# lambdaclass/lambda_elliptic_curves

Hardware: AMD Instinct MI355X
Metric: NTT elems/sec (Stark252 radix-2, 2^24, forward, bit-exact vs CPU: see 'bit_exact') [+ MSM G1 point-adds/sec under 'msm'] (higher is better)
Workload: dtype u32x8 (256-bit Montgomery, 32-bit limbs)

## Files before the change

### lambda_elliptic_curves_amd/csrc/field.cuh

```cuda
#pragma once
#include <stdint.h>

#if defined(__HIPCC__)
#include <hip/hip_runtime.h>
#define LW_HD __host__ __device__ __forceinline__
#else
#define LW_HD inline
#endif

namespace lw {

struct Stark252 {
    static constexpr int N = 8;
    static constexpr bool LAZY = true;
    static constexpr uint32_t INV = 0xffffffffu;
    static constexpr uint32_t TWO_ADICITY = 192;
    LW_HD static constexpr uint32_t p(int i) {
        constexpr uint32_t t[N] = {0x00000001u, 0x00000000u, 0x00000000u, 0x00000000u, 0x00000000u, 0x00000000u, 0x00000011u, 0x08000000u};
        return t[i];
    }
    LW_HD static constexpr uint32_t one(int i) {
        constexpr uint32_t t[N] = {0xffffffe1u, 0xffffffffu, 0xffffffffu, 0xffffffffu, 0xffffffffu, 0xffffffffu, 0xfffffdf0u, 0x07ffffffu};
        return t[i];
    }
// ... 273 lines not shown
    for (int i = 0; i < M + 2; i++) t[i] = 0;
    uint64_t z = (uint64_t)(0u - F::INV);
    z *= 2 - P[0] * z;
    const uint64_t inv = 0 - z;
    for (int i = 0; i < M; i++) {
        u128 c = 0;
        for (int j = 0; j < M; j++) {
            c += (u128)A[j] * B[i] + t[j];
            t[j] = (uint64_t)c;
            c >>= 64;
        }
        c += t[M];
        t[M] = (uint64_t)c;
        t[M + 1] = (uint64_t)(c >> 64);
        const uint64_t m = t[0] * inv;
        c = ((u128)m * P[0] + t[0]) >> 64;
        for (int j = 1; j < M; j++) {
            c += (u128)m * P[j] + t[j];
            t[j - 1] = (uint64_t)c;
            c >>= 64;
        }
        c += t[M];
        t[M - 1] = (uint64_t)c;
        t[M] = t[M + 1] + (uint64_t)(c >> 64);
    }
    Fe<F> r;
    for (int i = 0; i < M; i++) {
        r.v[2 * i] = (uint32_t)t[i];
        r.v[2 * i + 1] = (uint32_t)(t[i] >> 32);
    }
    return reduce_once<F>(r);
}
#endif

#if defined(__HIP_DEVICE_COMPILE__)
#define LW_MAC_V(A, B) "v_mad_u64_u32 %0, vcc, " A ", " B ", %0\n\tv_addc_co_u32_e32 %1, vcc, 0, %1, vcc\n\t"

__device__ __forceinline__ void mac96_x1(uint64_t &lo, uint32_t &hi, uint32_t a0, uint32_t b0) {
    asm(LW_MAC_V("%2", "%3") : "+v"(lo), "+v"(hi) : "v"(a0), "v"(b0) : "vcc");
}
__device__ __forceinline__ void mac96_x2(uint64_t &lo, uint32_t &hi, uint32_t a0, uint32_t b0, uint32_t a1, uint32_t b1) {
    asm(LW_MAC_V("%2", "%3") LW_MAC_V("%4", "%5") : "+v"(lo), "+v"(hi) : "v"(a0), "v"(b0), "v"(a1), "v"(b1) : "vcc");
}
__device__ __forceinline__ void mac96_x4(uint64_t &lo, uint32_t &hi, uint32_t a0, uint32_t b0, uint32_t a1, uint32_t b1,
                                         uint32_t a2, uint32_t b2, uint32_t a3, uint32_t b3) {
    asm(LW_MAC_V("%2", "%3") LW_MAC_V("%4", "%5") LW_MAC_V("%6", "%7") LW_MAC_V("%8", "%9")
        : "+v"(lo), "+v"(hi)
        : "v"(a0), "v"(b0), "v"(a1), "v"(b1), "v"(a2), "v"(b2), "v"(a3), "v"(b3)
        : "vcc");
}
#define LW_MAC_FIRST(A, B, INIT) "v_mad_u64_u32 %0, vcc, " A ", " B ", " INIT "\n\tv_addc_co_u32_e64 %1, vcc, 0, 0, vcc\n\t"
template <uint32_t C>
__device__ __forceinline__ void mac96_c1(uint64_t &lo, uint32_t &hi, uint32_t m0) {
    if constexpr (C == 0) {
    } else if constexpr (C <= 64) {
        asm(LW_MAC_V("%2", "%3") : "+v"(lo), "+v"(hi) : "v"(m0), "n"(C) : "vcc");
    } else {
        asm(LW_MAC_V("%2", "%3") : "+v"(lo), "+v"(hi) : "v"(m0), "s"(C) : "vcc");
    }
}
template <uint32_t C0, uint32_t C1, uint32_t C2, uint32_t C3>
__device__ __forceinline__ void mac96_s4(uint64_t &lo, uint32_t &hi, uint32_t m0, uint32_t m1, uint32_t m2, uint32_t m3) {
    asm(LW_MAC_V("%2", "%3") LW_MAC_V("%4", "%5") LW_MAC_V("%6", "%7") LW_MAC_V("%8", "%9")
        : "+v"(lo), "+v"(hi)
        : "v"(m0), "s"(C0), "v"(m1), "s"(C1), "v"(m2), "s"(C2), "v"(m3), "s"(C3)
        : "vcc");
}

template <class F, int K, int I, int IEND>
__device__ __forceinline__ void col_ab(uint64_t &lo, uint32_t &hi, const Fe<F> &a, const Fe<F> &b) {
    if constexpr (I + 4 <= IEND) {
        mac96_x4(lo, hi, a.v[I], b.v[K - I], a.v[I + 1], b.v[K - I - 1], a.v[I + 2], b.v[K - I - 2], a.v[I + 3], b.v[K - I - 3]);
        col_ab<F, K, I + 4, IEND>(lo, hi, a, b);
    } else if constexpr (I + 2 <= IEND) {
        mac96_x2(lo, hi, a.v[I], b.v[K - I], a.v[I + 1], b.v[K - I - 1]);
        col_ab<F, K, I + 2, IEND>(lo, hi, a, b);
    } else if constexpr (I + 1 <= IEND) {
        mac96_x1(lo, hi, a.v[I], b.v[K - I]);
    }
}
template <uint32_t C>
constexpr bool lw_is_literal() { return C > 64; }
template <class F, int K, int I, int IEND>
__device__ __forceinline__ void col_mp(uint64_t &lo, uint32_t &hi, const uint32_t (&m)[F::N]) {
    if constexpr (I + 4 <= IEND) {
        if constexpr (lw_is_literal<F::p(K - I)>() && lw_is_literal<F::p(K - I - 1)>() && lw_is_literal<F::p(K - I - 2)>() &&
                      lw_is_literal<F::p(K - I - 3)>()) {
            mac96_s4<F::p(K - I), F::p(K - I - 1), F::p(K - I - 2), F::p(K - I - 3)>(lo, hi, m[I], m[I + 1], m[I + 2], m[I + 3]);
            col_mp<F, K, I + 4, IEND>(lo, hi, m);
        } else {
            mac96_c1<F::p(K - I)>(lo, hi, m[I]);
            col_mp<F, K, I + 1, IEND>(lo, hi, m);
        }
    } else if constexpr (I + 1 <= IEND) {
        mac96_c1<F::p(K - I)>(lo, hi, m[I]);
        col_mp<F, K, I + 1, IEND>(lo, hi, m);
    }
}
template <class F>
struct lw_fused_columns {
    static constexpr bool value = false;
};
template <class F, int K, bool A_LT_P>
struct FusedCol;
template <class F, int K>
struct FusedColS;
#include "mac_chains.inc"

template <class F, int LO, int HI>
constexpr bool lw_all_literal() {
    for (int i = LO; i < HI; i++)
        if (F::p(i) <= 64) return false;
    return true;
}

template <class F, int P, int K>
__device__ __forceinline__ void fips_col(uint64_t init, const Fe<F> *const (&a)[P], const Fe<F> *const (&b)[P], uint32_t (&m)[F::N],
                                         uint32_t (&t)[F::N]) {
    constexpr int N = F::N;
    if constexpr (K == 2 * N - 1) {
        t[N - 1] = (uint32_t)init;
    } else {
        uint64_t lo;
        uint32_t hi;
        if constexpr (K < N) {
            col_ab_first_dispatch<F, K, 0, K + 1>(lo, hi, init, *a[0], *b[0]);
            if constexpr (P > 1) col_ab<F, K, 0, K + 1>(lo, hi, *a[1], *b[1]);
            if constexpr (P > 2) col_ab<F, K, 0, K + 1>(lo, hi, *a[2], *b[2]);
            if constexpr (P > 3) col_ab<F, K, 0, K + 1>(lo, hi, *a[3], *b[3]);
            if constexpr (K >= 1 && lw_all_literal<F, 1, K + 1>()) col_mp_dispatch<F, K, 0, K>(lo, hi, m);
            else col_mp<F, K, 0, K>(lo, hi, m);
            uint32_t mk;
            if constexpr (F::INV == 0xffffffffu) mk = 0u - (uint32_t)lo;
            else mk = (uint32_t)lo * F::INV;
            m[K] = mk;
            mac96_c1<F::p(0)>(lo, hi, mk);
        } else {
            col_ab_first_dispatch<F, K, K - N + 1, 2 * N - 1 - K>(lo, hi, init, *a[0], *b[0]);
            if constexpr (P > 1) col_ab<F, K, K - N + 1, N>(lo, hi, *a[1], *b[1]);
            if constexpr (P > 2) col_ab<F, K, K - N + 1, N>(lo, hi, *a[2], *b[2]);
            if constexpr (P > 3) col_ab<F, K, K - N + 1, N>(lo, hi, *a[3], *b[3]);
            if constexpr (lw_all_literal<F, K - N + 1, N>()) col_mp_dispatch<F, K, K - N + 1, 2 * N - 1 - K>(lo, hi, m);
            else col_mp<F, K, K - N + 1, N>(lo, hi, m);
            t[K - N] = (uint32_t)lo;
        }
        fips_col<F, P, K + 1>((lo >> 32) | ((uint64_t)hi << 32), a, b, m, t);
    }
}
__device__ __forceinline__ void lw_redc_unit(uint32_t &m, uint32_t &mid, uint32_t &top, uint32_t t, uint32_t w1, uint32_t w2) {
    asm("v_sub_co_u32_e32 %0, vcc, 0, %3\n\t"
        "v_addc_co_u32_e32 %1, vcc, 0, %4, vcc\n\t"
        "v_addc_co_u32_e32 %2, vcc, 0, %5, vcc"
        : "=&v"(m), "=&v"(mid), "=v"(top)
        : "v"(t), "v"(w1), "v"(w2)
        : "vcc");
}
__device__ __forceinline__ void lw_redc_unit0(uint32_t &m, uint32_t &mid, uint32_t &top, uint32_t t, uint32_t w1) {
    asm("v_sub_co_u32_e32 %0, vcc, 0, %3\n\t"
        "v_addc_co_u32_e32 %1, vcc, 0, %4, vcc\n\t"
        "v_addc_co_u32_e64 %2, vcc, 0, 0, vcc"
        : "=&v"(m), "=&v"(mid), "=v"(top)
        : "v"(t), "v"(w1)
        : "vcc");
}
template <class F, int K, bool A_LT_P, bool A_SGPR = false>
__device__ __forceinline__ void fips_fused(uint64_t init, const Fe<F> &a, const Fe<F> &b, uint32_t (&m)[F::N], uint32_t (&t)[F::N]) {
    constexpr int N = F::N;
    static_assert(F::p(0) == 1u && F::INV == 0xffffffffu, "fused columns need a unit low limb of the modulus");
    if constexpr (K == 2 * N - 1) {
        t[N - 1] = (uint32_t)init;
    } else {
        uint64_t lo;
        uint32_t hi;
        static_assert(A_LT_P || !A_SGPR, "the scalar-operand columns exist for a < p only");
        if constexpr (A_SGPR) FusedColS<F, K>::run(lo, hi, init, a, b, m);
        else FusedCol<F, K, A_LT_P>::run(lo, hi, init, a, b, m);
        if constexpr (K < N) {
            uint32_t mid, top;
            if constexpr (K == 0) lw_redc_unit0(m[0], mid, top, (uint32_t)lo, (uint32_t)(lo >> 32));
            else lw_redc_unit(m[K], mid, top, (uint32_t)lo, (uint32_t)(lo >> 32), hi);
            fips_fused<F, K + 1, A_LT_P, A_SGPR>(((uint64_t)top << 32) | mid, a, b, m, t);
        } else {
            t[K - N] = (uint32_t)lo;
            fips_fused<F, K + 1, A_LT_P, A_SGPR>((lo >> 32) | ((uint64_t)hi << 32), a, b, m, t);
        }
    }
}
template <class F, bool A_LT_P = false, bool A_SGPR = false>
__device__ __forceinline__ void fips_product(const Fe<F> &a, const Fe<F> &b, uint32_t (&t)[F::N]) {
    uint32_t m[F::N];
    if constexpr (lw_fused_columns<F>::value) {
        fips_fused<F, 0, A_LT_P, A_SGPR>(0ull, a, b, m, t);
    } else {
        const Fe<F> *const pa[1] = {&a}, *const pb[1] = {&b};
        fips_col<F, 1, 0>(0ull, pa, pb, m, t);
    }
}
template <class F>
__device__ __forceinline__ Fe<F> fe_mul_gfx9(const Fe<F> &a, const Fe<F> &b) {
    constexpr int N = F::N;
    uint32_t t[N];
    fips_product<F>(a, b, t);
    Fe<F> r;
#pragma unroll
    for (int i = 0; i < N; i++) r.v[i] = t[i];
    return reduce_once<F>(r);
}
#endif

template <class F>
LW_HD Fe<F> fe_mul(const Fe<F> &a, const Fe<F> &b) {
#if defined(__HIP_DEVICE_COMPILE__)
    return fe_mul_gfx9<F>(a, b);
#elif defined(LW_HOST_MUL64)
    return fe_mul_host64<F>(a, b);
#else
    return fe_mul_portable<F>(a, b);
#endif
}

template <class F>
LW_HD Fe<F> fe_sqr(const Fe<F> &a) { return fe_mul<F>(a, a); }

template <class F>
LW_HD Fe<F> fe_neg_raw(const Fe<F> &a) {
    uint32_t pk[F::N];
    limbs_kp<F, 0>(pk);
    Fe<F> r;
    limbs_sub<F::N>(r.v, pk, a.v);
    return r;
}
template <class F>
LW_HD Fe<F> fe_neg_raw_2p(const Fe<F> &a) {
    uint32_t pk[F::N];
    limbs_kp<F, 1>(pk);
    Fe<F> r;
    limbs_sub<F::N>(r.v, pk, a.v);
    return r;
}
template <class F, int P, int KSUM = P>
LW_HD Fe<F> fe_dot(const Fe<F> *const (&a)[P], const Fe<F> *const (&b)[P]) {
    static_assert(P >= 1 && P <= 4, "fe_dot: 1..4 products");
    static_assert(KSUM >= P, "fe_dot: KSUM counts every product at least once");
    static_assert((uint64_t)KSUM * ((uint64_t)F::p(F::N - 1) + 1) <= (1ull << 32), "fe_dot: sum of products would exceed 2p after reduction");
#if defined(__HIP_DEVICE_COMPILE__)
    constexpr int N = F::N;
    uint32_t m[N], t[N];
    fips_col<F, P, 0>(0ull, a, b, m, t);
    Fe<F> r;
#pragma unroll
    for (int i = 0; i < N; i++) r.v[i] = t[i];
    return reduce_once<F>(r);
#else
    static_assert(KSUM == P, "fe_dot: unreduced operands are a device-code feature");
    Fe<F> acc = fe_mul<F>(reduce_once<F>(*a[0]), *b[0]);
    for (int q = 1; q < P; q++) acc = fe_add<F>(acc, fe_mul<F>(reduce_once<F>(*a[q]), *b[q]));
    return acc;
#endif
}

template <class F, int LOGK>
LW_HD Fe<F> fe_cond_sub_kp(const Fe<F> &a) {
    constexpr int N = F::N;
    uint32_t kp[N];
    limbs_kp<F, LOGK>(kp);
    Fe<F> d;
    const uint32_t borrow = limbs_sub<N>(d.v, a.v, kp);
    Fe<F> r;
#pragma unroll
    for (int i = 0; i < N; i++) r.v[i] = borrow ? a.v[i] : d.v[i];
    return r;
}
LW_HD Fe<Stark252> fe_reduce_full(const Fe<Stark252> &x) {
    const uint32_t q = x.v[7] >> 27;
    const uint32_t z = lw_k(0u);
    const uint32_t sub[8] = {q, z, z, z, z, z, 17u * q, q << 27};
    Fe<Stark252> d;
    const uint32_t borrow = limbs_sub<8>(d.v, x.v, sub);
    uint32_t pm[8];
    limbs_p_masked<Stark252>(pm, 0u - borrow);
    Fe<Stark252> r;
    limbs_add<8>(r.v, d.v, pm);
    return r;
}
template <class F>
LW_HD Fe<F> fe_reduce_full(const Fe<F> &x) { return reduce_once<F>(x); }

template <class F>
LW_HD Fe<F> fe_add_raw(const Fe<F> &a, const Fe<F> &b) {
    Fe<F> s;
    limbs_add<F::N>(s.v, a.v, b.v);
    return s;
}
template <class F>
LW_HD Fe<F> fe_add2p_sub_raw(const Fe<F> &a, const Fe<F> &b) {
    constexpr int N = F::N;
    uint32_t kp[N];
    limbs_kp<F, 1>(kp);
    Fe<F> d, r;
    limbs_sub<N>(d.v, a.v, b.v);
    limbs_add<N>(r.v, d.v, kp);
    return r;
}
template <class F>
LW_HD Fe<F> fe_mul_lazy(const Fe<F> &a, const Fe<F> &b) {
#if defined(__HIP_DEVICE_COMPILE__)
    constexpr int N = F::N;
    uint32_t t[N];
    fips_product<F, true>(a, b, t);
    Fe<F> r;
#pragma unroll
    for (int i = 0; i < N; i++) r.v[i] = t[i];
    return r;
#else
    return fe_mul_portable_raw<F>(a, b);
#endif
}
template <class F>
LW_HD Fe<F> fe_mul_lazy_uniform(const Fe<F> &a, const Fe<F> &b) {
#if defined(__HIP_DEVICE_COMPILE__)
    constexpr int N = F::N;
    uint32_t t[N];
    fips_product<F, true, lw_fused_columns<F>::value>(a, b, t);
    Fe<F> r;
#pragma unroll
    for (int i = 0; i < N; i++) r.v[i] = t[i];
    return r;
#else
    return fe_mul_portable_raw<F>(a, b);
#endif
}

template <class F>
LW_HD Fe<F> fe_pow_u64(Fe<F> base, uint64_t e) {
    Fe<F> r = Fe<F>::one();
    while (e) {
        if (e & 1) r = fe_mul<F>(r, base);
        base = fe_sqr<F>(base);
        e >>= 1;
    }
    return r;
}

template <class F>
LW_HD Fe<F> fe_inv(const Fe<F> &a) {
    constexpr int N = F::N;
    uint32_t e[N];
    uint64_t borrow = 2;
#pragma unroll
    for (int i = 0; i < N; i++) {
        uint64_t t = (uint64_t)F::p(i) - borrow;
        e[i] = (uint32_t)t;
        borrow = (t >> 32) & 1;
    }
    Fe<F> r = Fe<F>::one();
    for (int i = N - 1; i >= 0; i--) {
        for (int bit = 31; bit >= 0; bit--) {
            r = fe_sqr<F>(r);
            if ((e[i] >> bit) & 1) r = fe_mul<F>(r, a);
        }
    }
    return r;
}

template <class F>
LW_HD constexpr int fe_modulus_bits() {
    int top = 0;
    for (int b = 0; b < 32; b++)
        if ((F::p(F::N - 1) >> b) & 1u) top = b + 1;
    return 32 * (F::N - 1) + top;
}
template <int N>
LW_HD uint32_t bingcd_update_ab(uint32_t (&x)[N], uint32_t (&y)[N], int32_t f, int32_t g, int32_t h, int32_t k) {
    int64_t cx = 0, cy = 0;
    uint32_t wx[N + 1], wy[N + 1];
#pragma unroll
    for (int i = 0; i < N; i++) {
        const int64_t zx = (int64_t)x[i] * f + (int64_t)y[i] * g + cx;
        const int64_t zy = (int64_t)x[i] * h + (int64_t)y[i] * k + cy;
        wx[i] = (uint32_t)zx;
        wy[i] = (uint32_t)zy;
        cx = zx >> 32;
        cy = zy >> 32;
    }
    wx[N] = (uint32_t)cx;
    wy[N] = (uint32_t)cy;
    const uint32_t nx = (uint32_t)((uint64_t)cx >> 63), ny = (uint32_t)((uint64_t)cy >> 63);
    uint32_t carx = nx, cary = ny;
#pragma unroll
    for (int i = 0; i < N; i++) {
        uint32_t rx = (wx[i] >> 30) | (wx[i + 1] << 2), ry = (wy[i] >> 30) | (wy[i + 1] << 2);
        rx ^= 0u - nx;
        ry ^= 0u - ny;
        const uint32_t sx = rx + carx, sy = ry + cary;
        carx = sx < rx ? 1u : 0u;
        cary = sy < ry ? 1u : 0u;
        x[i] = sx;
        y[i] = sy;
    }
    return nx | (ny << 1);
}
template <class F>
LW_HD void bingcd_update_uv(uint32_t (&u)[F::N], uint32_t (&v)[F::N], int32_t f, int32_t g, int32_t h, int32_t k) {
    constexpr int N = F::N;
    const uint32_t fu = ((uint32_t)(u[0] * (uint32_t)f + v[0] * (uint32_t)g) * F::INV) & 0x3fffffffu;
    const uint32_t fv = ((uint32_t)(u[0] * (uint32_t)h + v[0] * (uint32_t)k) * F::INV) & 0x3fffffffu;
    int64_t cu = 0, cv = 0;
    uint32_t wu[N + 1], wv[N + 1];
#pragma unroll
    for (int i = 0; i < N; i++) {
        const int64_t zu = (int64_t)u[i] * f + (int64_t)v[i] * g + (int64_t)((uint64_t)F::p(i) * fu) + cu;
        const int64_t zv = (int64_t)u[i] * h + (int64_t)v[i] * k + (int64_t)((uint64_t)F::p(i) * fv) + cv;
        wu[i] = (uint32_t)zu;
        wv[i] = (uint32_t)zv;
        cu = zu >> 32;
        cv = zv >> 32;
    }
    wu[N] = (uint32_t)cu;
    wv[N] = (uint32_t)cv;
    const uint32_t nu = (uint32_t)((uint64_t)cu >> 63), nv = (uint32_t)((uint64_t)cv >> 63);
    uint32_t ru[N], rv[N];
#pragma unroll
    for (int i = 0; i < N; i++) {
        ru[i] = (wu[i] >> 30) | (wu[i + 1] << 2);
        rv[i] = (wv[i] >> 30) | (wv[i + 1] << 2);
    }
    uint32_t pk[N], du[N], dv[N], su[N], sv[N];
#pragma unroll
    for (int i = 0; i < N; i++) pk[i] = F::p(i);
    const uint32_t bu = limbs_sub<N>(du, ru, pk), bv = limbs_sub<N>(dv, rv, pk);
    limbs_add<N>(su, ru, pk);
    limbs_add<N>(sv, rv, pk);
#pragma unroll
    for (int i = 0; i < N; i++) {
        u[i] = nu ? su[i] : (bu ? ru[i] : du[i]);
        v[i] = nv ? sv[i] : (bv ? rv[i] : dv[i]);
    }
}
template <class F>
LW_HD Fe<F> fe_inv_int_bingcd(const Fe<F> &y) {
    constexpr int N = F::N;
    constexpr int ROUNDS = (2 * fe_modulus_bits<F>()) / 29 + 2;
    uint32_t a[N], b[N], u[N], v[N];
#pragma unroll
    for (int i = 0; i < N; i++) {
        a[i] = y.v[i];
        b[i] = F::p(i);
        u[i] = i == 0 ? 1u : 0u;
        v[i] = 0u;
    }
#pragma nounroll
    for (int round = 0; round < ROUNDS; round++) {
        uint32_t a0 = 0, a1 = 0, b0 = 0, b1 = 0, c0 = 0xffffffffu, c1 = 0xffffffffu;
#pragma unroll
        for (int j = N - 1; j >= 0; j--) {
            const uint32_t aw = a[j], bw = b[j];
            a0 ^= (a0 ^ aw) & c0;
            a1 ^= (a1 ^ aw) & c1;
            b0 ^= (b0 ^ bw) & c0;
            b1 ^= (b1 ^ bw) & c1;
            c1 = c0;
            c0 &= ((aw | bw) == 0u) ? 0xffffffffu : 0u;
        }
        a1 |= a0 & c1;
        a0 &= ~c1;
        b1 |= b0 & c1;
        b0 &= ~c1;
        uint64_t a_hi = ((uint64_t)a0 << 32) | a1, b_hi = ((uint64_t)b0 << 32) | b1;
        uint32_t a_lo = a[0], b_lo = b[0];
        int32_t pa = 1, pb = 0, qa = 0, qb = 1;
#pragma unroll 2
        for (int i = 0; i < 30; i++) {
            const uint32_t r = a_hi > b_hi ? 1u : 0u;
            const uint32_t oa = (a_lo >> i) & 1u, ob = (b_lo >> i) & 1u;
            const uint32_t cAB = oa & ob & r, cBA = oa & ob & (r ^ 1u), cA = cAB | (oa ^ 1u);
            const uint32_t mAB = 0u - cAB, mBA = 0u - cBA, mA = 0u - cA;
            a_lo -= b_lo & mAB;
            a_hi -= b_hi & (uint64_t)(int64_t)(int32_t)mAB;
            pa -= qa & (int32_t)mAB;
            pb -= qb & (int32_t)mAB;
            b_lo -= a_lo & mBA;
            b_hi -= a_hi & (uint64_t)(int64_t)(int32_t)mBA;
            qa -= pa & (int32_t)mBA;
            qb -= pb & (int32_t)mBA;
            a_lo += a_lo & ~mA;
            pa += pa & (int32_t)~mA;
            pb += pb & (int32_t)~mA;
            a_hi = cA ? (a_hi >> 1) : a_hi;
            b_lo += b_lo & mA;
            qa += qa & (int32_t)mA;
            qb += qb & (int32_t)mA;
            b_hi = cA ? b_hi : (b_hi >> 1);
        }
        const uint32_t neg = bingcd_update_ab<N>(a, b, pa, pb, qa, qb);
        if (neg & 1u) { pa = -pa; pb = -pb; }
        if (neg & 2u) { qa = -qa; qb = -qb; }
        bingcd_update_uv<F>(u, v, pa, pb, qa, qb);
    }
    Fe<F> r;
    const bool zero = y.is_zero();
#pragma unroll
    for (int i = 0; i < N; i++) r.v[i] = zero ? 0u : (u[i] | v[i]);
    return r;
}
template <class F>
LW_HD Fe<F> fe_inv_fast(const Fe<F> &a) {
    const Fe<F> r3 = fe_mul<F>(Fe<F>::r2(), Fe<F>::r2());
    return fe_mul<F>(fe_inv_int_bingcd<F>(a), r3);
}

template <class F>
LW_HD Fe<F> fe_to_mont(const Fe<F> &a) { return fe_mul<F>(a, Fe<F>::r2()); }
template <class F>
LW_HD Fe<F> fe_from_mont(const Fe<F> &a) {
    Fe<F> o = Fe<F>::zero();
    o.v[0] = 1;
    return fe_mul<F>(a, o);
}
template <class F>
LW_HD Fe<F> fe_from_u64(uint64_t x) {
    Fe<F> o = Fe<F>::zero();
    o.v[0] = (uint32_t)x;
    o.v[1] = (uint32_t)(x >> 32);
    return fe_to_mont<F>(o);
}

template <class F>
LW_HD constexpr int mem_index(int k) { return 2 * (F::N / 2 - 1 - k / 2) + (k & 1); }

template <class F>
LW_HD Fe<F> fe_load(const void *ptr) {
    constexpr int N = F::N;
    const uint4 *q = reinterpret_cast<const uint4 *>(ptr);
    uint32_t m[N];
#pragma unroll
    for (int i = 0; i < N / 4; i++) {
        uint4 x = q[i];
        m[4 * i + 0] = x.x; m[4 * i + 1] = x.y; m[4 * i + 2] = x.z; m[4 * i + 3] = x.w;
    }
    Fe<F> r;
#pragma unroll
    for (int k = 0; k < N; k++) r.v[k] = m[mem_index<F>(k)];
    return r;
}
template <class F>
LW_HD void fe_store(void *ptr, const Fe<F> &a) {
    constexpr int N = F::N;
    uint32_t m[N];
#pragma unroll
    for (int k = 0; k < N; k++) m[mem_index<F>(k)] = a.v[k];
    uint4 *q = reinterpret_cast<uint4 *>(ptr);
#pragma unroll
    for (int i = 0; i < N / 4; i++) q[i] = make_uint4(m[4 * i], m[4 * i + 1], m[4 * i + 2], m[4 * i + 3]);
}

struct BabyBear {
    static constexpr uint32_t P = 2013265921u;
    static constexpr uint32_t MU = 0x88000001u;
    static constexpr uint32_t R2 = 0x45dddde3u;
    static constexpr uint32_t ONE = 0x0ffffffeu;
    static constexpr uint32_t TWO_ADICITY = 24;
    static constexpr uint32_t ROOT = 21;
};

LW_HD uint32_t bb_reduce(uint64_t x) {
    const uint32_t m = (uint32_t)x * (0u - BabyBear::MU);
    const uint32_t r = (uint32_t)((x + (uint64_t)m * BabyBear::P) >> 32);
    const uint32_t d = r - BabyBear::P;
    return d < r ? d : r;
}
LW_HD uint32_t bb_mul(uint32_t a, uint32_t b) { return bb_reduce((uint64_t)a * b); }
LW_HD uint32_t bb_add(uint32_t a, uint32_t b) {
    const uint32_t s = a + b, d = s - BabyBear::P;
    return d < s ? d : s;
}
LW_HD uint32_t bb_sub(uint32_t a, uint32_t b) {
    const uint32_t d = a - b, e = d + BabyBear::P;
    return e < d ? e : d;
}
LW_HD uint32_t bb_pow(uint32_t a, uint64_t e) {
    uint32_t r = BabyBear::ONE;
    while (e) {
        if (e & 1) r = bb_mul(r, a);
        a = bb_mul(a, a);
        e >>= 1;
    }
    return r;
}
LW_HD uint32_t bb_inv(uint32_t a) { return bb_pow(a, (uint64_t)BabyBear::P - 2); }
LW_HD uint32_t bb_from_r64(uint64_t w) { return bb_reduce(w); }
LW_HD uint64_t bb_to_r64(uint32_t v) { return (uint64_t)bb_mul(v, BabyBear::R2); }

}
```

### lambda_elliptic_curves_amd/csrc/ntt_kernels.cuh

```cuda
#pragma once
#include "field.cuh"

namespace lw {

constexpr int NTT_TILE_LOG = 11;
constexpr int NTT_TILE = 1 << NTT_TILE_LOG;
constexpr int NTT_THREADS = 512;
constexpr int NTT_KMAX = 2;
constexpr int NTT_LTW = 256;

struct NttPassParams {
    const uint4 *in;
    uint4 *out;
    const uint4 *tw;
    uint64_t in_batch_stride;
    uint64_t out_batch_stride;
    uint32_t L;
    uint32_t s0;
    uint32_t r;
    uint32_t logC;
    uint32_t nsteps;
    uint32_t k[8];
    const uint4 *cos_lo, *cos_hi;
    uint32_t cos_hbits;
    uint32_t cos_in;
    uint32_t cos_out;
    uint64_t in_mask;
    uint32_t lazy_in;
    uint32_t wave_sync;
    uint32_t scale;
    uint32_t sc[8];
};

__device__ __forceinline__ uint32_t bitrev_bits(uint32_t x, uint32_t bits) {
    return bits ? (__brev(x) >> (32 - bits)) : 0u;
}

template <class F>
__device__ __forceinline__ Fe<F> tw_load(const uint4 *tw, uint64_t g) {
    uint4 a = tw[2 * g], b = tw[2 * g + 1];
    Fe<F> r;
    r.v[0] = a.x; r.v[1] = a.y; r.v[2] = a.z; r.v[3] = a.w;
    r.v[4] = b.x; r.v[5] = b.y; r.v[6] = b.z; r.v[7] = b.w;
    return r;
}
template <class F>
__device__ __forceinline__ Fe<F> tw_load_uniform(const uint4 *tw, uint64_t g) {
    typedef const __attribute__((address_space(4))) uint32_t *const_words;
    const_words w = (const_words)(uintptr_t)(tw + 2 * g);
    Fe<F> r;
#pragma unroll
    for (int i = 0; i < 8; i++) r.v[i] = w[i];
    return r;
}
template <class F>
__device__ __forceinline__ void tw_store(uint4 *tw, uint64_t g, const Fe<F> &x) {
    tw[2 * g] = make_uint4(x.v[0], x.v[1], x.v[2], x.v[3]);
    tw[2 * g + 1] = make_uint4(x.v[4], x.v[5], x.v[6], x.v[7]);
}

template <class F>
__device__ __forceinline__ Fe<F> unpack_mem(uint4 q0, uint4 q1) {
    Fe<F> r;
    r.v[6] = q0.x; r.v[7] = q0.y; r.v[4] = q0.z; r.v[5] = q0.w;
    r.v[2] = q1.x; r.v[3] = q1.y; r.v[0] = q1.z; r.v[1] = q1.w;
    return r;
}
template <class F>
__device__ __forceinline__ void pack_mem(const Fe<F> &a, uint4 &q0, uint4 &q1) {
    q0 = make_uint4(a.v[6], a.v[7], a.v[4], a.v[5]);
    q1 = make_uint4(a.v[2], a.v[3], a.v[0], a.v[1]);
}

template <bool WL>
__device__ __forceinline__ uint32_t lds_slot(uint32_t m, uint32_t c, uint32_t r, uint32_t logC) {
    if (!WL) return (m << logC) | c;
    const uint32_t sw = r >= 4 ? ((5u * ((m >> 4) & 3u)) ^ ((c & 7u) << 1)) : 0u;
    return (c << r) | (m ^ sw);
}
__device__ __forceinline__ void lds_wave_sync() {
    __builtin_amdgcn_fence(__ATOMIC_RELEASE, "wavefront");
    __builtin_amdgcn_wave_barrier();
    __builtin_amdgcn_fence(__ATOMIC_ACQUIRE, "wavefront");
}

struct NttItemGeo {
    uint32_t c, mbase, m_high, sh;
    uint32_t hi_c;
    uint64_t gbase;
};
template <int K, bool LAST, bool WL, int FX>
__device__ __forceinline__ NttItemGeo ntt_item_geo(const NttPassParams &p, uint32_t w, uint32_t step, uint32_t t0, uint64_t base,
                                                   uint32_t hi_uniform, uint32_t hi_low) {
    const uint32_t r = FX ? (uint32_t)FX : p.r, logC = FX ? (uint32_t)(NTT_TILE_LOG - FX) : p.logC, L = p.L;
    NttItemGeo g;
    g.sh = r - t0 - K;
    uint32_t mr;
    if ((LAST && step == 0) || (WL && (LAST || step > 0))) {
        mr = w & ((1u << (r - K)) - 1);
        g.c = w >> (r - K);
    } else {
        g.c = w & ((1u << logC) - 1);
        mr = w >> logC;
    }
    const uint32_t m_low = mr & ((1u << g.sh) - 1);
    g.m_high = mr >> g.sh;
    g.mbase = (g.m_high << (g.sh + K)) | m_low;
    g.hi_c = hi_uniform;
    g.gbase = base;
    if (LAST) {
        g.hi_c = (bitrev_bits(g.c, logC) << (L - r - logC)) | hi_low;
        g.gbase = (uint64_t)g.hi_c << r;
    }
    return g;
}

__device__ __forceinline__ void ntt_tw_stage_load(const NttPassParams &p, uint32_t r, uint32_t hi_uniform, uint4 &tq0, uint4 &tq1) {
    const uint32_t ti = threadIdx.x;
    if (ti + 1 < (1u << r)) {
        const uint32_t t = 31 - __clz(ti + 1), xg = ti + 1 - (1u << t);
        const uint64_t g = ((uint64_t)hi_uniform << t) | xg;
        tq0 = p.tw[2 * g];
        tq1 = p.tw[2 * g + 1];
    }
}
__device__ __forceinline__ void ntt_tw_stage_store(uint4 (*ltw)[NTT_LTW], uint32_t r, const uint4 &tq0, const uint4 &tq1) {
    const uint32_t ti = threadIdx.x;
    if (ti + 1 < (1u << r)) {
        ltw[0][ti] = tq0;
        ltw[1][ti] = tq1;
    }
}

template <class F, int K, bool LAST, bool EXTRA>
__device__ __forceinline__ void ntt_load_global(const NttPassParams &p, const NttItemGeo &g, const uint4 *gin, uint32_t lgS, Fe<F> *x) {
    constexpr int E = 1 << K;
#pragma unroll
    for (int j = 0; j < E; j++) {
        const uint32_t m = g.mbase | ((uint32_t)j << g.sh);
        const uint64_t e = (LAST ? (g.gbase + m) : (g.gbase + ((uint64_t)m << lgS) + g.c)) & p.in_mask;
        x[j] = unpack_mem<F>(gin[2 * e], gin[2 * e + 1]);
    }
    if (EXTRA && p.cos_in) {
#pragma unroll
        for (int j = 0; j < E; j++) {
            const uint32_t m = g.mbase | ((uint32_t)j << g.sh);
            const uint64_t e = (LAST ? (g.gbase + m) : (g.gbase + ((uint64_t)m << lgS) + g.c)) & p.in_mask;
            Fe<F> pw = fe_mul<F>(tw_load<F>(p.cos_lo, e & ((1ull << p.cos_hbits) - 1)), tw_load<F>(p.cos_hi, e >> p.cos_hbits));
            x[j] = fe_mul<F>(x[j], pw);
        }
    }
}

template <class F, bool LAST, bool WL>
__device__ __forceinline__ Fe<F> ntt_fetch_tw(const NttPassParams &p, const NttItemGeo &g, uint4 (*ltw)[NTT_LTW], uint32_t t0, int q) {
    const int u = 31 - __builtin_clz(q + 1), jt = q + 1 - (1 << u);
    Fe<F> tw;
    if (LAST || WL) {
        const uint64_t gt = ((uint64_t)g.hi_c << (t0 + u)) | ((uint64_t)g.m_high << u);
        tw = tw_load<F>(p.tw, gt | (uint32_t)jt);
    } else {
        const uint32_t li = (1u << (t0 + u)) - 1 + ((g.m_high << u) | (uint32_t)jt);
        uint4 a = ltw[0][li], b = ltw[1][li];
        tw.v[0] = a.x; tw.v[1] = a.y; tw.v[2] = a.z; tw.v[3] = a.w;
        tw.v[4] = b.x; tw.v[5] = b.y; tw.v[6] = b.z; tw.v[7] = b.w;
    }
    return tw;
}

template <class F, int K, bool LAST, bool WL, bool PF, bool UNI = false>
__device__ __forceinline__ void ntt_butterflies(const NttPassParams &p, const NttItemGeo &g, uint4 (*ltw)[NTT_LTW], uint32_t t0, bool first,
                                                Fe<F> *x) {
    constexpr int E = 1 << K;
    static_assert(!UNI || (!LAST && !WL), "wave-uniform twiddles: plain non-last passes only");
    const uint32_t m_high = UNI ? (uint32_t)__builtin_amdgcn_readfirstlane((int)g.m_high) : g.m_high;
    if (F::LAZY && first && p.lazy_in) {
#pragma unroll
        for (int j = 0; j < E / 2; j++) x[j] = fe_reduce_full(x[j]);
    }

    auto fetch_tw = [&](int q) -> Fe<F> { return ntt_fetch_tw<F, LAST, WL>(p, g, ltw, t0, q); };
    Fe<F> tw_next, tw_uni[E - 1];
    if (UNI) {
#pragma unroll
        for (int q = 0; q < E - 1; q++) {
            const int u = 31 - __builtin_clz(q + 1), jt = q + 1 - (1 << u);
            tw_uni[q] = tw_load_uniform<F>(p.tw, ((uint64_t)g.hi_c << (t0 + u)) | ((uint64_t)m_high << u) | (uint32_t)jt);
        }
    } else if (PF) {
        tw_next = fetch_tw(0);
    }
#pragma unroll
    for (int q = 0; q < E - 1; q++) {
        const int u = 31 - __builtin_clz(q + 1), jt = q + 1 - (1 << u);
        const int half = 1 << (K - 1 - u);
        const Fe<F> tw = UNI ? tw_uni[q] : PF ? tw_next : fetch_tw(q);
        if (!UNI && PF && q + 1 < E - 1) tw_next = fetch_tw(q + 1);
        const bool unit = (jt == 0) && (g.hi_c == 0) && (m_high == 0);
#pragma unroll
        for (int jl = 0; jl < half; jl++) {
            const int j = (jt << (K - u)) | jl;
            if (F::LAZY) {
                Fe<F> wb = unit ? fe_reduce_full(x[j + half]) : UNI ? fe_mul_lazy_uniform<F>(tw, x[j + half]) : fe_mul_lazy<F>(tw, x[j + half]);
                Fe<F> a = x[j];
                x[j] = fe_add_raw<F>(a, wb);
                x[j + half] = fe_add2p_sub_raw<F>(a, wb);
            } else {
                Fe<F> wb = unit ? x[j + half] : fe_mul<F>(tw, x[j + half]);
                Fe<F> a = x[j];
                x[j] = fe_add<F>(a, wb);
                x[j + half] = fe_sub<F>(a, wb);
            }
            __builtin_amdgcn_sched_barrier(0);
        }
    }
}

template <class F, int K, bool LAST, bool EXTRA, int FX>
__device__ __forceinline__ void ntt_finish(const NttPassParams &p, const NttItemGeo &g, Fe<F> *x) {
    constexpr int E = 1 << K;
    const uint32_t r = FX ? (uint32_t)FX : p.r, logC = FX ? (uint32_t)(NTT_TILE_LOG - FX) : p.logC, L = p.L;
    if (EXTRA && LAST && p.cos_out) {
#pragma unroll
        for (int j = 0; j < E; j++) {
            const uint32_t m = g.mbase | ((uint32_t)j << g.sh);
            const uint64_t i_nat = ((uint64_t)bitrev_bits(m, r) << (L - r)) + ((uint64_t)blockIdx.x << logC) + g.c;
            Fe<F> pw = fe_mul<F>(tw_load<F>(p.cos_lo, i_nat & ((1ull << p.cos_hbits) - 1)), tw_load<F>(p.cos_hi, i_nat >> p.cos_hbits));
            if (F::LAZY) x[j] = fe_cond_sub_kp<F, 0>(fe_mul_lazy<F>(pw, x[j]));
            else x[j] = fe_mul<F>(x[j], pw);
        }
    } else if (EXTRA && p.scale) {
        Fe<F> sc;
#pragma unroll
        for (int i = 0; i < 8; i++) sc.v[i] = p.sc[i];
#pragma unroll
        for (int j = 0; j < E; j++) {
            if (F::LAZY) x[j] = fe_cond_sub_kp<F, 0>(fe_mul_lazy<F>(sc, x[j]));
            else x[j] = fe_mul<F>(x[j], sc);
        }
    } else if (F::LAZY && LAST) {
#pragma unroll
        for (int j = 0; j < E; j++) x[j] = fe_reduce_full(x[j]);
    }
}

template <class F, int K>
__device__ __forceinline__ void ntt_store_global(const NttItemGeo &g, uint4 *gout, uint32_t lgS, const Fe<F> *x) {
#pragma unroll
    for (int j = 0; j < (1 << K); j++) {
        const uint32_t m = g.mbase | ((uint32_t)j << g.sh);
        const uint64_t e = g.gbase + ((uint64_t)m << lgS) + g.c;
        uint4 q0, q1;
        pack_mem<F>(x[j], q0, q1);
        gout[2 * e] = q0;
        gout[2 * e + 1] = q1;
    }
}

template <class F, int K, bool LAST, bool EXTRA, bool WL, int FX = 0>
__device__ __forceinline__ void ntt_item(const NttPassParams &p, uint4 (*lds)[NTT_TILE], uint4 (*ltw)[NTT_LTW], const uint4 *gin,
                                         uint4 *gout, uint32_t w, uint32_t step, uint32_t t0, uint64_t base, uint32_t lgS,
                                         uint32_t hi_uniform, uint32_t hi_low, bool last_step, bool stage_tw) {
    constexpr int E = 1 << K;
    const uint32_t r = FX ? (uint32_t)FX : p.r, logC = FX ? (uint32_t)(NTT_TILE_LOG - FX) : p.logC;
    const NttItemGeo g = ntt_item_geo<K, LAST, WL, FX>(p, w, step, t0, base, hi_uniform, hi_low);
    uint4 tq0, tq1;
    if (!LAST && !WL && stage_tw) ntt_tw_stage_load(p, r, hi_uniform, tq0, tq1);
    Fe<F> x[E];
    if (step == 0) {
        ntt_load_global<F, K, LAST, EXTRA>(p, g, gin, lgS, x);
    } else {
#pragma unroll
        for (int j = 0; j < E; j++) {
            const uint32_t idx = lds_slot<WL>(g.mbase | ((uint32_t)j << g.sh), g.c, r, logC);
            x[j] = unpack_mem<F>(lds[0][idx], lds[1][idx ^ (WL ? 1u : 0u)]);
        }
    }
    if (!LAST && !WL && stage_tw) {
        ntt_tw_stage_store(ltw, r, tq0, tq1);
        __syncthreads();
    }
    ntt_butterflies<F, K, LAST, WL, true>(p, g, ltw, t0, step == 0, x);
    if (last_step) ntt_finish<F, K, LAST, EXTRA, FX>(p, g, x);
    if (!LAST && last_step) {
        ntt_store_global<F, K>(g, gout, lgS, x);
        return;
    }
#pragma unroll
    for (int j = 0; j < E; j++) {
        const uint32_t idx = lds_slot<WL>(g.mbase | ((uint32_t)j << g.sh), g.c, r, logC);
        pack_mem<F>(x[j], lds[0][idx], lds[1][idx ^ (WL ? 1u : 0u)]);
    }
}

template <bool LAST, int FX>
constexpr bool ntt_one_plane() { return FX && !LAST; }
template <class F, bool LAST, bool EXTRA, int FX>
constexpr int ntt_waves_per_simd() { return ntt_one_plane<LAST, FX>() && F::LAZY && !EXTRA ? 6 : 4; }

template <class F>
__device__ __forceinline__ void ntt_exchange(uint4 *lds, const uint32_t (&so)[4], const uint32_t (&si)[4], Fe<F> *x) {
    uint4 o0[4], o1[4], n0[4];
#pragma unroll
    for (int j = 0; j < 4; j++) pack_mem<F>(x[j], o0[j], o1[j]);
#pragma unroll
    for (int j = 0; j < 4; j++) lds[so[j]] = o0[j];
    __syncthreads();
#pragma unroll
    for (int j = 0; j < 4; j++) n0[j] = lds[si[j]];
    __syncthreads();
#pragma unroll
    for (int j = 0; j < 4; j++) lds[so[j]] = o1[j];
    __syncthreads();
#pragma unroll
    for (int j = 0; j < 4; j++) x[j] = unpack_mem<F>(n0[j], lds[si[j]]);
}

template <int K, int FX>
__device__ __forceinline__ void ntt_item_slots(const NttItemGeo &g, uint32_t *s) {
#pragma unroll
    for (int j = 0; j < (1 << K); j++) s[j] = lds_slot<false>(g.mbase | ((uint32_t)j << g.sh), g.c, FX, NTT_TILE_LOG - FX);
}

template <class F, bool EXTRA, int FX>
__device__ __forceinline__ void ntt_tile_fx(const NttPassParams &p, uint4 *lds, uint4 (*ltw)[NTT_LTW], const uint4 *gin, uint4 *gout,
                                            uint64_t base, uint32_t lgS, uint32_t hi_uniform) {
    constexpr bool PF = ntt_waves_per_simd<F, false, EXTRA, FX>() < 6;
    static_assert(NTT_TILE_LOG - NTT_KMAX == 9 && NTT_THREADS == 512, "wave-uniform twiddles of steps 0 and 1 assume 512 radix-4 items");
    const uint32_t tid = threadIdx.x;
    Fe<F> x[4];
    uint32_t so[4], si[4];

    NttItemGeo g = ntt_item_geo<2, false, false, FX>(p, tid, 0u, 0u, base, hi_uniform, 0u);
    uint4 tq0, tq1;
    ntt_tw_stage_load(p, FX, hi_uniform, tq0, tq1);
    ntt_load_global<F, 2, false, EXTRA>(p, g, gin, lgS, x);
    ntt_tw_stage_store(ltw, FX, tq0, tq1);
    ntt_butterflies<F, 2, false, false, PF, true>(p, g, ltw, 0u, true, x);
    ntt_item_slots<2, FX>(g, so);
#pragma unroll
    for (uint32_t s = 1; s < FX / 2; s++) {
        g = ntt_item_geo<2, false, false, FX>(p, tid, s, 2 * s, base, hi_uniform, 0u);
        ntt_item_slots<2, FX>(g, si);
        ntt_exchange<F>(lds, so, si, x);
        if (s == 1) ntt_butterflies<F, 2, false, false, PF, true>(p, g, ltw, 2 * s, false, x);
        else ntt_butterflies<F, 2, false, false, PF>(p, g, ltw, 2 * s, false, x);
#pragma unroll
        for (int j = 0; j < 4; j++) so[j] = si[j];
    }
    if constexpr (FX % 2) {
        const NttItemGeo ga = ntt_item_geo<1, false, false, FX>(p, tid, FX / 2, FX - 1, base, hi_uniform, 0u);
        const NttItemGeo gb = ntt_item_geo<1, false, false, FX>(p, tid + NTT_THREADS, FX / 2, FX - 1, base, hi_uniform, 0u);
        ntt_item_slots<1, FX>(ga, si);
        ntt_item_slots<1, FX>(gb, si + 2);
        ntt_exchange<F>(lds, so, si, x);
        ntt_butterflies<F, 1, false, false, PF>(p, ga, ltw, FX - 1, false, x);
        ntt_butterflies<F, 1, false, false, PF>(p, gb, ltw, FX - 1, false, x + 2);
        ntt_finish<F, 1, false, EXTRA, FX>(p, ga, x);
        ntt_finish<F, 1, false, EXTRA, FX>(p, gb, x + 2);
        ntt_store_global<F, 1>(ga, gout, lgS, x);
        ntt_store_global<F, 1>(gb, gout, lgS, x + 2);
    } else {
        ntt_finish<F, 2, false, EXTRA, FX>(p, g, x);
        ntt_store_global<F, 2>(g, gout, lgS, x);
    }
}

template <class F, bool LAST, bool EXTRA, bool WL, int FX = 0>
__global__ __launch_bounds__(NTT_THREADS, (ntt_waves_per_simd<F, LAST, EXTRA, FX>())) void ntt_pass_kernel(NttPassParams p) {
    __shared__ uint4 lds[ntt_one_plane<LAST, FX>() ? 1 : 2][NTT_TILE];
    __shared__ uint4 ltw[LAST ? 1 : 2][LAST ? 1 : NTT_LTW];
    const uint32_t tid = threadIdx.x;
    static_assert(!FX || (NTT_TILE == 2048 && NTT_THREADS == 512 && (FX == 8 || FX == 7 || FX == 6)), "FX: 2^8 x 8, 2^7 x 16 or 2^6 x 32 rows x columns");
    static_assert(!WL || LAST, "the column layout is the last pass's");
    const uint32_t r = FX ? (uint32_t)FX : p.r, logC = FX ? (uint32_t)(NTT_TILE_LOG - FX) : p.logC, L = p.L;
    const uint32_t tile_log = r + logC;
    const uint4 *gin = p.in + 2 * (uint64_t)blockIdx.y * p.in_batch_stride;
    uint4 *gout = p.out + 2 * (uint64_t)blockIdx.y * p.out_batch_stride;
    const uint32_t b = blockIdx.x;

    uint64_t base = 0;
    uint32_t lgS = 0, hi_uniform = 0, hi_low = 0;
    if (!LAST) {
        lgS = L - p.s0 - r;
        const uint32_t lo_bits = lgS - logC;
        const uint32_t lo_blk = b & ((1u << lo_bits) - 1);
        hi_uniform = b >> lo_bits;
        base = ((uint64_t)hi_uniform << (L - p.s0)) + ((uint64_t)lo_blk << logC);
    } else {
        hi_low = bitrev_bits(b, L - r - logC);
    }

    if constexpr (ntt_one_plane<LAST, FX>()) {
        ntt_tile_fx<F, EXTRA, FX>(p, lds[0], (uint4 (*)[NTT_LTW])ltw, gin, gout, base, lgS, hi_uniform);
    } else {
    if constexpr (FX) {
#define LW_FX_STEP(S)                                                                                                                  \
    do {                                                                                                                                \
        if (S) {                                                                                                                        \
            if (WL && ((p.wave_sync >> (S)) & 1u)) lds_wave_sync();                                                                     \
            else __syncthreads();                                                                                                       \
        }                                                                                                                               \
        ntt_item<F, 2, LAST, EXTRA, WL, FX>(p, lds, (uint4 (*)[NTT_LTW])ltw, gin, gout, tid, (S), 2u * (S), base, lgS, hi_uniform, hi_low,    \
                                            2 * ((S) + 1) == FX, false);                                                                \
    } while (0)
        LW_FX_STEP(0u);
        LW_FX_STEP(1u);
        LW_FX_STEP(2u);
        if constexpr (FX == 8) LW_FX_STEP(3u);
        if constexpr (FX == 7) {
            __syncthreads();
            ntt_item<F, 1, LAST, EXTRA, WL, FX>(p, lds, (uint4 (*)[NTT_LTW])ltw, gin, gout, tid, 3u, 6u, base, lgS, hi_uniform, hi_low, true, false);
            ntt_item<F, 1, LAST, EXTRA, WL, FX>(p, lds, (uint4 (*)[NTT_LTW])ltw, gin, gout, tid + NTT_THREADS, 3u, 6u, base, lgS, hi_uniform, hi_low, true, false);
        }
#undef LW_FX_STEP
    } else {
    const bool stage_inside = !LAST && !WL && (1u << (tile_log - p.k[0])) >= (uint32_t)NTT_THREADS && (1u << r) <= (uint32_t)NTT_THREADS;
    if (!LAST && !WL && !stage_inside) {
        for (uint32_t i = tid; i + 1 < (1u << r); i += NTT_THREADS) {
            const uint32_t t = 31 - __clz(i + 1), x = i + 1 - (1u << t);
            const uint64_t g = ((uint64_t)hi_uniform << t) | x;
            ltw[0][i] = p.tw[2 * g];
            ltw[1][i] = p.tw[2 * g + 1];
        }
        __syncthreads();
    }
    uint32_t t0 = 0;
    for (uint32_t step = 0; step < p.nsteps; step++) {
        const uint32_t k = p.k[step];
        const uint32_t nitems = 1u << (tile_log - k);
        const bool last_step = (step + 1 == p.nsteps);
        if (step) {
            if (WL && ((p.wave_sync >> step) & 1u)) lds_wave_sync();
            else __syncthreads();
        }
        for (uint32_t w = tid; w < nitems; w += NTT_THREADS) {
            if (NTT_KMAX >= 3 && k == 3) ntt_item<F, (NTT_KMAX >= 3 ? 3 : 1), LAST, EXTRA, WL>(p, lds, (uint4 (*)[NTT_LTW])ltw, gin, gout, w, step, t0, base, lgS, hi_uniform, hi_low, last_step, stage_inside && step == 0 && w == tid);
            else if (k == 2) ntt_item<F, 2, LAST, EXTRA, WL>(p, lds, (uint4 (*)[NTT_LTW])ltw, gin, gout, w, step, t0, base, lgS, hi_uniform, hi_low, last_step, stage_inside && step == 0 && w == tid);
            else ntt_item<F, 1, LAST, EXTRA, WL>(p, lds, (uint4 (*)[NTT_LTW])ltw, gin, gout, w, step, t0, base, lgS, hi_uniform, hi_low, last_step, stage_inside && step == 0 && w == tid);
        }
        t0 += k;
    }
    }
    if constexpr (!LAST) return;
    __syncthreads();

    auto write_one = [&](uint32_t f) {
        const uint32_t e = f >> 1, plane = f & 1;
        const uint32_t c = e & ((1u << logC) - 1);
        const uint32_t m = e >> logC;
        const uint64_t g = ((uint64_t)bitrev_bits(m, r) << (L - r)) + ((uint64_t)b << logC) + c;
        gout[2 * g + plane] = lds[plane][lds_slot<WL>(m, c, r, logC) ^ (WL ? plane : 0u)];
    };
    if constexpr (FX) {
#pragma unroll
        for (int q = 0; q < 2 * NTT_TILE / NTT_THREADS; q++) write_one(tid + (uint32_t)q * NTT_THREADS);
    } else {
        const uint32_t total = 2u << tile_log;
        for (uint32_t f = tid; f < total; f += NTT_THREADS) write_one(f);
    }
    }
}

template <class F>
__global__ void twiddle_fill_kernel(uint4 *tw, const uint4 *lo, const uint4 *hi, uint32_t bits, uint32_t hbits,
                                    uint64_t count) {
    uint64_t g = (uint64_t)blockIdx.x * blockDim.x + threadIdx.x;
    if (g >= count) return;
    uint32_t e = bitrev_bits((uint32_t)g, bits);
    Fe<F> a = tw_load<F>(lo, e & ((1u << hbits) - 1));
    Fe<F> b = tw_load<F>(hi, e >> hbits);
    tw_store<F>(tw, g, fe_mul<F>(a, b));
}

struct FeWords8 {
    uint32_t w[8];
};
template <class F>
__global__ void power_tables_kernel(uint4 *lo, uint4 *hi, FeWords8 base, uint32_t hbits, uint64_t hi_count, FeWords8 scale, int has_scale) {
    const uint64_t t = (uint64_t)blockIdx.x * blockDim.x + threadIdx.x;
    const uint64_t lo_count = 1ull << hbits;
    if (t >= lo_count + hi_count) return;
    const bool is_lo = t < lo_count;
    const uint64_t e = is_lo ? t : ((t - lo_count) << hbits);
    Fe<F> b, r = Fe<F>::one();
#pragma unroll
    for (int k = 0; k < 8; k++) b.v[k] = base.w[k];
    for (int bit = 63 - (e ? __clzll((long long)e) : 63); bit >= 0; bit--) {
        r = fe_sqr<F>(r);
        if ((e >> bit) & 1) r = fe_mul<F>(r, b);
    }
    if (!is_lo && has_scale) {
        Fe<F> sc;
#pragma unroll
        for (int k = 0; k < 8; k++) sc.v[k] = scale.w[k];
        r = fe_mul<F>(r, sc);
    }
    if (is_lo) tw_store<F>(lo, t, r);
    else tw_store<F>(hi, t - lo_count, r);
}

}
```

Measured before the change: 14.06 billion.

## Add C·p offset on load so early lazy NTT stages skip 2p correction

For fixed-shape (FX) passes on Stark252, each element loaded by the first butterfly stage is given a constant multiple of p: the top-limb quotient is subtracted and C·p is added. The first nfree stages can then compute the butterfly difference as a plain a-b, without adding 2p, because a compile-time bound plan guarantees values stay nonnegative and below 2^256. This removes one 256-bit add per butterfly in those stages. In exchange, the load-time reduction becomes a subtract plus an add, and correctness now depends on the static bound analysis and on the downstream final reduction coping with larger intermediate multiples of p.

```diff
diff --git a/lambda_elliptic_curves_amd/csrc/field.cuh b/lambda_elliptic_curves_amd/csrc/field.cuh
--- a/lambda_elliptic_curves_amd/csrc/field.cuh
+++ b/lambda_elliptic_curves_amd/csrc/field.cuh
@@ -599,6 +599,44 @@
     limbs_add<N>(r.v, d.v, kp);
     return r;
 }
+template <int C>
+LW_HD void limbs_cp_stark(uint32_t (&k)[8]) {
+    static_assert(C >= 1 && C <= 15, "C*p limb by limb: 17C and C << 27 must fit their limbs");
+    const uint32_t z = lw_k(0u);
+    k[0] = lw_k((uint32_t)C); k[1] = z; k[2] = z; k[3] = z; k[4] = z; k[5] = z;
+    k[6] = lw_k(17u * (uint32_t)C); k[7] = lw_k((uint32_t)C << 27);
+}
+LW_HD Fe<Stark252> fe_sub_qp(const Fe<Stark252> &x) {
+    const uint32_t q = x.v[7] >> 27;
+    const uint32_t z = lw_k(0u);
+    const uint32_t sub[8] = {q, z, z, z, z, z, 17u * q, q << 27};
+    Fe<Stark252> d;
+    limbs_sub<8>(d.v, x.v, sub);
+    return d;
+}
+template <int C>
+LW_HD Fe<Stark252> fe_add_cp(const Fe<Stark252> &x) {
+    uint32_t cp[8];
+    limbs_cp_stark<C>(cp);
+    Fe<Stark252> r;
+    limbs_add<8>(r.v, x.v, cp);
+    return r;
+}
+template <int C>
+LW_HD Fe<Stark252> fe_reduce_offset(const Fe<Stark252> &x) { return fe_add_cp<C>(fe_sub_qp(x)); }
+template <class F, bool FREE>
+LW_HD void fe_butterfly_raw(Fe<F> &a, Fe<F> &t) {
+    const Fe<F> a0 = a;
+    a = fe_add_raw<F>(a0, t);
+    if (FREE) {
+        Fe<F> d;
+        limbs_sub<F::N>(d.v, a0.v, t.v);
+        t = d;
+    } else {
+        t = fe_add2p_sub_raw<F>(a0, t);
+    }
+}
+
 template <class F>
 LW_HD Fe<F> fe_mul_lazy(const Fe<F> &a, const Fe<F> &b) {
 #if defined(__HIP_DEVICE_COMPILE__)
diff --git a/lambda_elliptic_curves_amd/csrc/ntt_bound_plan.h b/lambda_elliptic_curves_amd/csrc/ntt_bound_plan.h
--- /dev/null
+++ b/lambda_elliptic_curves_amd/csrc/ntt_bound_plan.h
@@ -0,0 +1,40 @@
+#pragma once
+
+namespace lw {
+
+constexpr int NTT_LAZY_MAX_STAGES = 8;
+constexpr int NTT_LAZY_TOP_MULTIPLE = 31;
+
+struct NttBoundPlan {
+    int c;
+    int nfree;
+};
+
+constexpr bool ntt_bound_plan_holds(int r, NttBoundPlan b) {
+    if (b.c < 1 || b.nfree < 0 || b.nfree > r) return false;
+    for (int s = 0; s < b.nfree; s++)
+        if (b.c - 1 - 2 * s < 2) return false;
+    return b.c + 1 + 2 * r <= NTT_LAZY_TOP_MULTIPLE;
+}
+
+constexpr NttBoundPlan ntt_bound_plan(int r) {
+    for (int nfree = r; nfree > 0; nfree--) {
+        const NttBoundPlan b = {2 * nfree + 1, nfree};
+        if (ntt_bound_plan_holds(r, b)) return b;
+    }
+    return NttBoundPlan{1, 0};
+}
+
+constexpr bool ntt_bound_plans_hold() {
+    for (int r = 1; r <= NTT_LAZY_MAX_STAGES; r++)
+        if (!ntt_bound_plan_holds(r, ntt_bound_plan(r))) return false;
+    return true;
+}
+static_assert(ntt_bound_plans_hold(), "lazy NTT pass: a free stage below 2p or a value at 2^256");
+static_assert(ntt_bound_plan(8).c == 13 && ntt_bound_plan(8).nfree == 6, "8 stages: 13p on load, stages 0-5 free");
+static_assert(ntt_bound_plan(7).c == 15 && ntt_bound_plan(7).nfree == 7, "7 stages: 15p on load, all free");
+static_assert(ntt_bound_plan(6).c == 13 && ntt_bound_plan(6).nfree == 6, "6 stages: 13p on load, all free");
+static_assert(!ntt_bound_plan_holds(8, NttBoundPlan{15, 7}) && !ntt_bound_plan_holds(8, NttBoundPlan{14, 7}),
+              "8 stages with seven free: 14p starts too low, 15p ends at 32p");
+
+}
diff --git a/lambda_elliptic_curves_amd/csrc/ntt_kernels.cuh b/lambda_elliptic_curves_amd/csrc/ntt_kernels.cuh
--- a/lambda_elliptic_curves_amd/csrc/ntt_kernels.cuh
+++ b/lambda_elliptic_curves_amd/csrc/ntt_kernels.cuh
@@ -1,5 +1,6 @@
 #pragma once
 #include "field.cuh"
+#include "ntt_bound_plan.h"
 
 namespace lw {
 
@@ -168,13 +169,24 @@
     return tw;
 }
 
-template <class F, int K, bool LAST, bool WL, bool PF, bool UNI = false>
+template <class F, int K, bool LAST, bool WL, bool PF, bool UNI = false, int FX = 0>
 __device__ __forceinline__ void ntt_butterflies(const NttPassParams &p, const NttItemGeo &g, uint4 (*ltw)[NTT_LTW], uint32_t t0, bool first,
                                                 Fe<F> *x) {
     constexpr int E = 1 << K;
     static_assert(!UNI || (!LAST && !WL), "wave-uniform twiddles: plain non-last passes only");
     const uint32_t m_high = UNI ? (uint32_t)__builtin_amdgcn_readfirstlane((int)g.m_high) : g.m_high;
-    if (F::LAZY && first && p.lazy_in) {
+    constexpr bool OFFSET = F::LAZY && FX != 0;
+    constexpr NttBoundPlan BP = ntt_bound_plan(FX ? FX : 1);
+    if constexpr (OFFSET) {
+        if (first) {
+            if (p.lazy_in) {
+#pragma unroll
+                for (int j = 0; j < E / 2; j++) x[j] = fe_sub_qp(x[j]);
+            }
+#pragma unroll
+            for (int j = 0; j < E / 2; j++) x[j] = fe_add_cp<BP.c>(x[j]);
+        }
+    } else if (F::LAZY && first && p.lazy_in) {
 #pragma unroll
         for (int j = 0; j < E / 2; j++) x[j] = fe_reduce_full(x[j]);
     }
@@ -197,14 +209,15 @@
         const Fe<F> tw = UNI ? tw_uni[q] : PF ? tw_next : fetch_tw(q);
         if (!UNI && PF && q + 1 < E - 1) tw_next = fetch_tw(q + 1);
         const bool unit = (jt == 0) && (g.hi_c == 0) && (m_high == 0);
+        const bool free_stage = OFFSET && t0 + (uint32_t)u < (uint32_t)BP.nfree;
 #pragma unroll
         for (int jl = 0; jl < half; jl++) {
             const int j = (jt << (K - u)) | jl;
             if (F::LAZY) {
                 Fe<F> wb = unit ? fe_reduce_full(x[j + half]) : UNI ? fe_mul_lazy_uniform<F>(tw, x[j + half]) : fe_mul_lazy<F>(tw, x[j + half]);
-                Fe<F> a = x[j];
-                x[j] = fe_add_raw<F>(a, wb);
-                x[j + half] = fe_add2p_sub_raw<F>(a, wb);
+                if (free_stage) fe_butterfly_raw<F, true>(x[j], wb);
+                else fe_butterfly_raw<F, false>(x[j], wb);
+                x[j + half] = wb;
             } else {
                 Fe<F> wb = unit ? x[j + half] : fe_mul<F>(tw, x[j + half]);
                 Fe<F> a = x[j];
@@ -280,7 +293,7 @@
         ntt_tw_stage_store(ltw, r, tq0, tq1);
         __syncthreads();
     }
-    ntt_butterflies<F, K, LAST, WL, true>(p, g, ltw, t0, step == 0, x);
+    ntt_butterflies<F, K, LAST, WL, true, false, FX>(p, g, ltw, t0, step == 0, x);
     if (last_step) ntt_finish<F, K, LAST, EXTRA, FX>(p, g, x);
     if (!LAST && last_step) {
         ntt_store_global<F, K>(g, gout, lgS, x);
@@ -336,15 +349,15 @@
     ntt_tw_stage_load(p, FX, hi_uniform, tq0, tq1);
     ntt_load_global<F, 2, false, EXTRA>(p, g, gin, lgS, x);
     ntt_tw_stage_store(ltw, FX, tq0, tq1);
-    ntt_butterflies<F, 2, false, false, PF, true>(p, g, ltw, 0u, true, x);
+    ntt_butterflies<F, 2, false, false, PF, true, FX>(p, g, ltw, 0u, true, x);
     ntt_item_slots<2, FX>(g, so);
 #pragma unroll
     for (uint32_t s = 1; s < FX / 2; s++) {
         g = ntt_item_geo<2, false, false, FX>(p, tid, s, 2 * s, base, hi_uniform, 0u);
         ntt_item_slots<2, FX>(g, si);
         ntt_exchange<F>(lds, so, si, x);
-        if (s == 1) ntt_butterflies<F, 2, false, false, PF, true>(p, g, ltw, 2 * s, false, x);
-        else ntt_butterflies<F, 2, false, false, PF>(p, g, ltw, 2 * s, false, x);
+        if (s == 1) ntt_butterflies<F, 2, false, false, PF, true, FX>(p, g, ltw, 2 * s, false, x);
+        else ntt_butterflies<F, 2, false, false, PF, false, FX>(p, g, ltw, 2 * s, false, x);
 #pragma unroll
         for (int j = 0; j < 4; j++) so[j] = si[j];
     }
@@ -354,8 +367,8 @@
         ntt_item_slots<1, FX>(ga, si);
         ntt_item_slots<1, FX>(gb, si + 2);
         ntt_exchange<F>(lds, so, si, x);
-        ntt_butterflies<F, 1, false, false, PF>(p, ga, ltw, FX - 1, false, x);
-        ntt_butterflies<F, 1, false, false, PF>(p, gb, ltw, FX - 1, false, x + 2);
+        ntt_butterflies<F, 1, false, false, PF, false, FX>(p, ga, ltw, FX - 1, false, x);
+        ntt_butterflies<F, 1, false, false, PF, false, FX>(p, gb, ltw, FX - 1, false, x + 2);
         ntt_finish<F, 1, false, EXTRA, FX>(p, ga, x);
         ntt_finish<F, 1, false, EXTRA, FX>(p, gb, x + 2);
         ntt_store_global<F, 1>(ga, gout, lgS, x);
```

Measured after the change: 14.42 billion, median of 6. +2.5%, better.
